# 77even/Fast-nnUNet

Hardware: AMD Instinct MI355X
Metric: 3d_fullres patches/sec (distilled r=2 student, sliding window, one 512^3 CT; volume resident in HBM at step start; step ends with: fp16 logits resident in HBM) (higher is better)
Workload: dtype f16

## Files before the change

fast-nnunet_amd/csrc/conv3d.hip:

```cpp
#include "fnn_device.h"
#include "conv_common.h"
#include <cstdlib>

template <int NB>
__global__ __launch_bounds__(256) void conv3d_mfma_kernel(const ConvParams p) {
    extern __shared__ __attribute__((aligned(16))) char smem[];
    const int tid = threadIdx.x, lane = tid & 63, wave = tid >> 6;

    int t = blockIdx.x;
    const int tw = t % p.tiles_w; t /= p.tiles_w;
    const int th = t % p.tiles_h; t /= p.tiles_h;
    const int td = t % p.tiles_d;
    const int n = t / p.tiles_d;
    const int cb0 = blockIdx.y * NB;

    const int od0 = td * FNN_TILE_D, oh0 = th * FNN_TILE_H, ow0 = tw * FNN_TILE_W;
    const int ID = (FNN_TILE_D - 1) * p.sd + p.kd;
    const int IH = (FNN_TILE_H - 1) * p.sh + p.kh;
    const int IW = (FNN_TILE_W - 1) * p.sw + p.kw;
    const int IVOX = ID * IH * IW;
    const int T = p.kd * p.kh * p.kw;
    const int cin_total = p.chunks * 16;

    char *sA = smem;
// ... 865 lines not shown
                for (int wres = 1; wres >= 0; --wres) {
                    if (!wres && !(p.ksteps == 5 || (p.ksteps == 14 && mb == 8))) continue;
                    const size_t lds = persist_lds_bytes(p, nb, mb, wres != 0);
                    const int per_cu = (int)((160 * 1024) / lds);
                    if (per_cu < 2) continue;
                    const int wpc = per_cu > 3 ? 3 : per_cu;
                    if (wres && mb == 8 && p.ksteps == 5 && (p.chunks == 1 || p.chunks == 2)) {
                        const int ivox4 = (3 * p.sd + p.kd) * ((FNN_TILE_H - 1) * p.sh + p.kh) * ((FNN_TILE_W - 1) * p.sw + p.kw);
                        if (ivox4 * 2 <= 4 * 256 && persist_lds_bytes(p, 1, 4, true) * 3 <= 160 * 1024) {
                            set_persist(c, 1, 4, 1, 5, p.chunks, 4, 0, 3);
                            return true;
                        }
                    }
                    set_persist(c, 1, mb, wres, p.ksteps == 5 ? 5 : wres ? 0 : 14, 0, 8, 0, wpc);
                    return true;
                }
            }
        }
        if (p.ksteps <= 14) {
            set_ldsk(c, nb, mbsel, 8);
            return true;
        }
    }
    if (!o.conv_v1 && s2_choose(p, c)) return true;
    if (!o.conv_v1 && p.ksteps <= 14) {
        const int nbs = (p.Cout / 16) % 2 == 0 ? 2 : 1;
        const int ID = (2 - 1) * p.sd + p.kd, IH = (FNN_TILE_H - 1) * p.sh + p.kh, IW = (FNN_TILE_W - 1) * p.sw + p.kw;
        const long long tiles = (long long)plan_n * ((p.Do + 1) / 2) * p.tiles_h * p.tiles_w;
        const int groups = (p.Cout / 16) / nbs;
        if (nbs == 2 && ID * IH * IW * 2 <= 12 * 256 && persist_lds_bytes(p, 2, 2, false, false, 12) <= 80 * 1024 &&
            tiles >= 8LL * (512 / groups) && 512 / groups >= 8 && p.chunks == 1 && persist_lds_bytes(p, 2, 2, true, true, 12) <= 80 * 1024) {
            set_persist(c, 2, 2, 1, 0, 1, 12, 1, 2);
            c.gx = 512 / groups;
            return true;
        }
        if (ID * IH * IW * 2 <= 16 * 256 && ldsk_lds_bytes(p, nbs, 2) <= 80 * 1024) {
            set_ldsk(c, nbs, 2, ID * IH * IW * 2 <= 8 * 256 ? 8 : 16);
            return true;
        }
    }
    if (nb == 4 && conv3d_lds_bytes(p, 4) > 160 * 1024) nb = 2;
    if (conv3d_lds_bytes(p, nb) > 160 * 1024) return false;
    c.kernel = CK_NB; c.t[0] = nb;
    snprintf(c.name, sizeof c.name, "conv3d_mfma_kernel<%d> (generic fallback)", nb);
    return true;
}

ConvOverrides ConvOverrides::from_env() {
    ConvOverrides o;
    o.conv_v1 = fnn_knob("FNN_CONV_V1") != nullptr;
    o.no_row = fnn_knob("FNN_NO_ROW") != nullptr;
    o.no_stem_row = fnn_knob("FNN_NO_STEM_ROW") != nullptr;
    o.no_zr6 = fnn_knob("FNN_NO_ZR6") != nullptr;
    o.no_zq12 = fnn_knob("FNN_NO_ZQ12") != nullptr;
    o.no_zsw = fnn_knob("FNN_NO_ZSW") != nullptr;
    o.no_zp = fnn_knob("FNN_NO_ZP") != nullptr;
    o.zp_no_half = fnn_knob("FNN_ZP_NO_HALF") != nullptr;
    o.zps_no_half = fnn_knob("FNN_ZPS_NO_HALF") != nullptr;
    if (const char *v = fnn_knob("FNN_ZR_MIN_WGS")) o.zr_min_wgs = atoi(v);
    if (const char *v = fnn_knob("FNN_FP8_LEVELS")) o.fp8_levels = atoi(v);
    return o;
}

bool conv_choose(const ThinParams &tp, const ConvOverrides &o, ConvChoice &c) {
    c = ConvChoice{};
    if (tp.fuse) {
        ConvChoice t;
        if (!thin_choose(tp, t)) return false;
        if (!row_choose(tp, o, c)) c = t;
        return true;
    }
    const ConvParams &p = tp.c;
    const unsigned long long out_item = 2ull * p.Do * p.Ho * p.Wo * p.Cout;
    unsigned long long in_item = 0;
    for (int i = 0; i < p.n_src; ++i) {
        const unsigned long long b = 2ull * p.Di * p.Hi * p.Wi * p.src[i].C;
        in_item = b > in_item ? b : in_item;
    }
    if (out_item >= (1ull << 31) || in_item >= (1ull << 32) || (long long)p.Di * p.Hi >= (1 << 24) || p.Wi >= (1 << 24)) return false;
    if (zp_choose(p, o, c) || zr_choose(p, o, c)) return true;
    c = ConvChoice{};
    return row_choose(tp, o, c) || conv_choose_linear(p, o, c);
}

int launch_conv(const ThinParams &tp_in, const ConvChoice &c, hipStream_t st) {
    if (c.kernel == CK_ROW_STEM && tp_in.Y * tp_in.Z >= (1ll << 30)) {
        ConvChoice t;
        return thin_choose(tp_in, t) ? launch_conv(tp_in, t, st) : -1;
    }
    fnn_note_kernel("%s", c.name);
    ThinParams tp = tp_in;
    ConvParams &p = tp.c;
    p.tile_d = FNN_TILE_D;
    p.tiles_d = (p.Do + FNN_TILE_D - 1) / FNN_TILE_D;
    p.tiles_h = (p.Ho + FNN_TILE_H - 1) / FNN_TILE_H;
    p.tiles_w = (p.Wo + FNN_TILE_W - 1) / FNN_TILE_W;
    switch (c.kernel) {
        case CK_ZS: case CK_ZSP: case CK_ZSW: case CK_ZR: case CK_ZR8: case CK_ZQ12: case CK_ZR12: case CK_ZRW:
            return launch_conv3d_zr(p, c, st);
        case CK_ZP: case CK_ZPS: return launch_conv2d_zp(p, c, st);
        case CK_ROW: case CK_ROW_STEM: return launch_conv_row(tp, c, st);
        case CK_THIN: return launch_conv_thin(tp, c, st);
        case CK_PERSIST: return launch_persist(p, c, st);
        case CK_LDSK:
            if (c.t[1] == 2) {
                if (c.t[2] == 8) return c.t[0] == 2 ? launch_ldsk<2, 2, 8>(p, st) : launch_ldsk<1, 2, 8>(p, st);
// ... 10 lines not shown
```

fast-nnunet_amd/csrc/conv3d_zr.hip:

```cpp
#include "fnn_device.h"
#include "conv_common.h"
#include <type_traits>
#include <cstdlib>

int conv3d_ksteps(int packing, int taps) { return packing == FNN_PACK_ZR ? 15 : packing == FNN_PACK_ZP ? 9 : (taps + 1) / 2; }

int conv3d_kstep_tap(int packing, int ks, int half, int taps) {
    if (packing == FNN_PACK_ZR) {
        const int pr = ks / 3, dz = ks % 3, t = 2 * pr + half;
        return t < 9 ? dz * 9 + t : -1;
    }
    const int t = 2 * ks + half;
    return t < taps ? t : -1;
}

int conv3d_pack_cout(int packing, int nblk, int cb, int m) {
    if ((packing != FNN_PACK_ZR && packing != FNN_PACK_ZP) || nblk % 2 != 0) return cb * 16 + m;
    return (cb >> 1) * 32 + (m >> 2) * 8 + (cb & 1) * 4 + (m & 3);
}

bool zr_choose(const ConvParams &p, const ConvOverrides &o, ConvChoice &c) {
    if (p.kd != 3 || p.kh != 3 || p.kw != 3 || p.sd != 1) return false;
    const int nblk = p.Cout / 16;
    const int plan_n = p.plan_N > 0 ? p.plan_N : p.N;
    c.packing = FNN_PACK_ZR; c.ksteps = 15; c.chunks = p.chunks;
    if (p.sh == 2 && p.sw == 2) {
        if (p.fp8 || nblk % 2 != 0 || (long long)p.Di * p.Hi * p.Wi >= (1 << 23) || p.Do < 8) return false;
        const int tiles_d = (p.Do + 7) / 8, tiles_h = (p.Ho + 3) / 4, tiles_w = (p.Wo + 7) / 8, groups = nblk / 2;
        if ((long long)plan_n * tiles_d * tiles_h * tiles_w * (p.Cout / 32) < 768) return false;
        c.stats_slots = tiles_d * tiles_h * tiles_w;
        const bool persistent = p.chunks == 1 && p.n_src == 1 && plan_n * c.stats_slots >= 512 * 8;
        if (persistent && !o.no_zsw && tiles_d >= 4) {
            const long long cols = (long long)plan_n * tiles_h * tiles_w * groups;
            int segs = 1;
            while (cols * segs < 8 * 512 && segs * 2 <= tiles_d / 2) segs *= 2;
            c.tps = (tiles_d + segs - 1) / segs;
            c.segs = (tiles_d + c.tps - 1) / c.tps;
            c.kernel = CK_ZSW;
            snprintf(c.name, sizeof c.name, "conv3d_zsw_kernel");
        } else if (persistent) {
            c.gx = 512 / groups < 8 ? 8 : 512 / groups;
            c.kernel = CK_ZSP;
            snprintf(c.name, sizeof c.name, "conv3d_zsp_kernel");
        } else {
            c.kernel = CK_ZS; c.t[0] = 2;
            snprintf(c.name, sizeof c.name, "conv3d_zs_kernel<2>");
        }
        return true;
    }
    if (p.sh != 1 || p.sw != 1) return false;
    const long long vox = (long long)p.Do * p.Ho * p.Wo;
    if (vox >= (1 << 23)) return false;
    if (vox * 32 * (p.chunks > 0 ? p.chunks : 1) >= (1ll << 31) || vox * 2 * p.Cout >= (1ll << 31)) return false;
    const int nb = nblk % 2 == 0 ? 2 : 1;
    const int th = (p.Ho + 7) / 8, tw = (p.Wo + 7) / 8;
    if (nb == 2 && !p.fp8 && p.Ho <= 6 && p.Wo <= 8 && p.Do >= 10 && p.Do % 10 == 0 && !o.no_zr6 &&
        (long long)plan_n * (p.Do / 10) * (nblk / 2) >= 160) {
        c.stats_slots = ((p.Do + 9) / 10) * th * tw;
        c.kernel = CK_ZR; c.t[0] = 2; c.t[1] = 10; c.t[2] = 6;
        snprintf(c.name, sizeof c.name, "conv3d_zr_kernel<%d,%d,%d>", 2, 10, 6);
        return true;
    }
    int td = 8;
    while (td >= 4 && (p.Do < td || (long long)plan_n * ((p.Do + td - 1) / td) * th * tw * (nblk / nb) < o.zr_min_wgs)) td -= 4;
    if (td < 4) return false;
    c.stats_slots = ((p.Do + td - 1) / td) * th * tw;
    c.t[0] = nb; c.t[1] = td;
    if (p.fp8) {
        c.kernel = CK_ZR8;
        snprintf(c.name, sizeof c.name, "conv3d_zr8_kernel<%d,%d>", nb, td);
    } else if (nb == 2 && !o.no_zq12 && conv3d_zq12_fits(p, c.stats_slots)) {
        c.kernel = CK_ZQ12;
        snprintf(c.name, sizeof c.name, "conv3d_zq12_kernel");
    } else if (nb == 2 && p.Ho > 8 && p.Ho <= 12 && p.Wo > 8 && p.Wo <= 12 && c.stats_slots >= (p.Do + 3) / 4) {
        c.kernel = CK_ZR12; c.t[0] = 4;
        snprintf(c.name, sizeof c.name, "conv3d_zr12_kernel<%d>", 4);
    } else if (p.chunks == 1 && td == 8 && (p.Do + 7) / 8 >= 4) {
        const int tiles_d = (p.Do + 7) / 8;
        const long long cols = (long long)plan_n * th * tw * (nblk / nb);
        int segs = 1;
        while (cols * segs < 2 * 768 && segs * 2 <= tiles_d / 2) segs *= 2;
        c.tps = (tiles_d + segs - 1) / segs;
        c.segs = (tiles_d + c.tps - 1) / c.tps;
        c.kernel = CK_ZRW;
        snprintf(c.name, sizeof c.name, "conv3d_zrw_kernel<%d>", nb);
    } else {
        c.kernel = CK_ZR;
        snprintf(c.name, sizeof c.name, "conv3d_zr_kernel<%d,%d>", nb, td);
    }
    return true;
}

typedef int fnn_i32x4 __attribute__((ext_vector_type(4)));
template <int TD, bool BIAS = true>
static __device__ __forceinline__ void zr_epilogue_pair(const ConvParams &p, const f32x4 (&acc)[TD][2], const float4 (&bv)[2],
                                                        int n, int od0, int oh0, int ow0, int cb0, int wave, int lane,
                                                        float (&t1)[2][4], float (&t2)[2][4]) {
    const int q = lane >> 4, r = lane & 15;
    const unsigned item_bytes = (unsigned)p.Do * p.Ho * p.Wo * p.Cout * 2;
    const __amdgpu_buffer_rsrc_t rsrc = __builtin_amdgcn_make_buffer_rsrc(p.out + (size_t)n * (item_bytes >> 1), 0,
                                                                           item_bytes, 0x00020000);
    const unsigned ovs2 = (unsigned)FNN_OVS(p) * 2;
    const unsigned coff = (unsigned)(cb0 + (q >> 1)) * (unsigned)(FNN_OCS(p) * 2) + (unsigned)(q & 1) * 16;
    const int oh = oh0 + 2 * wave + (r >> 3), ow = ow0 + (r & 7);
    const bool ok_hw = oh < p.Ho && ow < p.Wo;
    const f16x2 ones = {(f16)1.f, (f16)1.f};
#pragma unroll
    for (int mb = 0; mb < TD; mb += 2) {
        f16x8 o[2];
#pragma unroll
        for (int h = 0; h < 2; ++h) {
            const int od = od0 + mb + h;
            const bool ok = ok_hw && od < p.Do;
            unsigned voff = ok ? (unsigned)((od * p.Ho + oh) * p.Wo + ow) * ovs2 + coff : 0x80000000u;
#ifdef FNN_TMODE
            if (p.tmode & 4) voff = 0x80000000u;
#endif
#pragma unroll
            for (int nb = 0; nb < 2; ++nb) {
                o[h][nb * 4 + 0] = (f16)(BIAS ? acc[mb + h][nb][0] + bv[nb].x : acc[mb + h][nb][0]);
                o[h][nb * 4 + 1] = (f16)(BIAS ? acc[mb + h][nb][1] + bv[nb].y : acc[mb + h][nb][1]);
                o[h][nb * 4 + 2] = (f16)(BIAS ? acc[mb + h][nb][2] + bv[nb].z : acc[mb + h][nb][2]);
                o[h][nb * 4 + 3] = (f16)(BIAS ? acc[mb + h][nb][3] + bv[nb].w : acc[mb + h][nb][3]);
            }
            __builtin_amdgcn_raw_buffer_store_b128(__builtin_bit_cast(fnn_i32x4, o[h]), rsrc, voff, 0, 0);
            if (!ok) o[h] = (f16x8){0, 0, 0, 0, 0, 0, 0, 0};
        }
#pragma unroll
        for (int nb = 0; nb < 2; ++nb)
#pragma unroll
            for (int j = 0; j < 4; ++j) {
                const f16x2 pr = {o[0][nb * 4 + j], o[1][nb * 4 + j]};
                t1[nb][j] = __builtin_amdgcn_fdot2(pr, ones, t1[nb][j], false);
                t2[nb][j] = __builtin_amdgcn_fdot2(pr, pr, t2[nb][j], false);
            }
    }
}

typedef unsigned fnn_u32x4v __attribute__((ext_vector_type(4)));
template <int NB, int TD, int TH = 8>
__global__ __launch_bounds__(TH * 32, 2) void conv3d_zr_kernel(const ConvParams p) {
    extern __shared__ __attribute__((aligned(16))) char smem[];
    const int tid = threadIdx.x, lane = tid & 63, wave = __builtin_amdgcn_readfirstlane(tid >> 6);
    FNN_STAMP_DECL
    FNN_STAMP();
    constexpr int NT = TH * 32;
    constexpr int IH = TH + 2, IW = 10, PW = 12, ID = TD + 2;
    constexpr int PS = IH * PW * 32;
    constexpr int ABYTES = ID * PS;
    constexpr int KS = 15;
    constexpr int WB = KS * 64;
    constexpr int WPB = (WB + NT - 1) / NT;
    static_assert(WB - (WPB - 1) * NT == 192, "the last weight element group covers exactly waves 0 .. 2");

    int t;
    {
        const int nwg = gridDim.x, bid = blockIdx.x;
        const int qd = nwg >> 3, rm = nwg & 7, xcd = bid & 7, idx = bid >> 3;
        t = __builtin_amdgcn_readfirstlane((xcd < rm ? xcd * (qd + 1) : rm * (qd + 1) + (xcd - rm) * qd) + idx);
    }
    const int tw = __builtin_amdgcn_readfirstlane(t % p.tiles_w); t = __builtin_amdgcn_readfirstlane(t / p.tiles_w);
    const int th = __builtin_amdgcn_readfirstlane(t % p.tiles_h); t = __builtin_amdgcn_readfirstlane(t / p.tiles_h);
    const int td = __builtin_amdgcn_readfirstlane(t % p.tiles_d);
    const int n = __builtin_amdgcn_readfirstlane(t / p.tiles_d);
    const int cb0 = blockIdx.y * NB;
    const int od0 = td * TD, oh0 = th * 8, ow0 = tw * 8;

    char *sA = smem;
    char *sW = smem + ABYTES;

    const int col = tid >> 1, cg = tid & 1;
    const int zh = (col * 205) >> 11, zw = col - zh * IW;
    const bool has_col = tid < 2 * IH * IW;
    const int gh = oh0 - 1 + zh, gw = ow0 - 1 + zw;
    const bool ok_hw = has_col & ((unsigned)gh < (unsigned)p.Hi) & ((unsigned)gw < (unsigned)p.Wi);
    const int hw_lin = __mul24(gh, p.Wi) + gw;
    const int ldso0 = (zh * PW + zw) * 32 + ((cg ^ (zh & 1)) * 16);
    const int wlds = ABYTES + tid * 16;
    unsigned pmask = (1u << ID) - 1;
    if (od0 == 0) pmask &= ~1u;
    {
        const int over = od0 + TD + 1 - p.Di;
        if (over > 0) pmask &= (1u << (ID - over)) - 1;
    }
    pmask = __builtin_amdgcn_readfirstlane(pmask);

    f32x4 acc[TD][NB];
    fnn_u32x4v xr[ID], wr[NB][WPB];
#ifdef FNN_NORM_FP32
    float scu[16], shu[16];
#else
    fnn_u32x4v ssv[2];
#endif
    float slope_next = 1.f;
#ifdef FNN_TMODE
    bool first_chunk = true;
#endif

    __amdgpu_buffer_rsrc_t rx, rw[NB];
    unsigned voff = 0x80000000u, plane_bytes = 0;
    auto prep = [&](int ch) {
        const int c_glob = ch * 16;
        const int s = (c_glob < p.src[0].C) ? 0 : 1;
        const int c_uni = c_glob - (s ? p.src[0].C : 0);
        const int sC = p.src[s].C;
        const int vs = FNN_VS(p.src[s]);
        const unsigned item_bytes = (unsigned)p.Di * p.Hi * p.Wi * sC * 2;
        const f16 *sp = p.src[s].ptr + (size_t)n * (item_bytes >> 1) + (c_uni >> 4) * FNN_CS(p.src[s]);
        rx = __builtin_amdgcn_make_buffer_rsrc((void *)sp, 0, item_bytes, 0x00020000);
        slope_next = p.src[s].slope;
#ifdef FNN_NORM_FP32
        const float *qs = p.src[s].ss ? p.src[s].ss + (size_t)(2 * n) * sC + c_uni : p.ident_ss + c_uni;
        const float *qh = p.src[s].ss ? qs + sC : p.ident_ss + 512 + c_uni;
#pragma unroll
        for (int j = 0; j < 16; ++j) { scu[j] = qs[j]; shu[j] = qh[j]; }
#else
        {
            const unsigned short *q = p.src[s].ssh ? p.src[s].ssh + ((size_t)n * sC + c_uni) * 2 : p.ident_ssh + c_uni * 2;
            const fnn_u32x4v *qv = (const fnn_u32x4v *)(q + cg * 16);
            ssv[0] = qv[0]; ssv[1] = qv[1];
        }
#endif
        voff = ok_hw ? (unsigned)hw_lin * (unsigned)(vs * 2) + cg * 16 : 0x80000000u;
        plane_bytes = (unsigned)p.Hi * p.Wi * vs * 2;
#pragma unroll
        for (int nb = 0; nb < NB; ++nb) {
            const f16 *wp = p.wpk + ((size_t)((cb0 + nb) * p.chunks + ch) * WB) * 8;
            rw[nb] = __builtin_amdgcn_make_buffer_rsrc((void *)wp, 0, WB * 16, 0x00020000);
        }
    };
#ifndef FNN_ZR_SLICES
#define FNN_ZR_SLICES 5
#endif
    constexpr int SL = FNN_ZR_SLICES;
    auto load_part = [&](int part) {
#pragma unroll
        for (int u = 0; u < ID; ++u) {
            if (u * SL / ID != part) continue;
            int gd = od0 - 1 + u;
            gd = gd < 0 ? 0 : (gd >= p.Di ? p.Di - 1 : gd);
            xr[u] = __builtin_bit_cast(fnn_u32x4v, __builtin_amdgcn_raw_buffer_load_b128(rx, voff, (unsigned)gd * plane_bytes, 0));
        }
#ifdef FNN_TMODE
        if ((p.tmode & 8) && !first_chunk) return;
#endif
#pragma unroll
        for (int e = 0; e < NB * WPB; ++e) {
            if (e * SL / (NB * WPB) != part) continue;
            const int nb = e / WPB, u = e % WPB;
            wr[nb][u] = __builtin_bit_cast(fnn_u32x4v, __builtin_amdgcn_raw_buffer_load_b128(rw[nb], tid * 16, u * (NT * 16), 0));
        }
    };
    auto commit = [&]() {
        const f16 slope_h = (f16)slope_next;
#ifdef FNN_NORM_FP32
        float sc[8], sh[8];
#pragma unroll
        for (int j = 0; j < 8; ++j) {
            sc[j] = ok_hw ? (cg ? scu[8 + j] : scu[j]) : 0.f;
            sh[j] = ok_hw ? (cg ? shu[8 + j] : shu[j]) : 0.f;
        }
#else
        const fnn_u32x4v zero4 = {0u, 0u, 0u, 0u};
        const f16x8 sc_h = __builtin_bit_cast(f16x8, ok_hw ? ssv[0] : zero4), sh_h = __builtin_bit_cast(f16x8, ok_hw ? ssv[1] : zero4);
#endif
        if (has_col) {
#pragma unroll
            for (int u = 0; u < ID; ++u) {
                const f16x8 x = __builtin_bit_cast(f16x8, xr[u]);
#ifdef FNN_NORM_FP32
                f16x8 o;
#pragma unroll
                for (int j = 0; j < 8; ++j) o[j] = (f16)fmaf((float)x[j], sc[j], sh[j]);
#else
                f16x8 o = x * sc_h + sh_h;
#endif
                o = __builtin_elementwise_max(o, o * slope_h);
                *(f16x8 *)(sA + ldso0 + u * PS) = o;
            }
            if (pmask != (1u << ID) - 1) {
                unsigned pm = pmask;
                asm volatile("" : "+s"(pm));
#pragma unroll
                for (int u = 0; u < ID; ++u)
                    if (!((pm >> u) & 1)) *(f16x8 *)(sA + ldso0 + u * PS) = (f16x8){0, 0, 0, 0, 0, 0, 0, 0};
            }
        }
#ifdef FNN_TMODE
        if ((p.tmode & 8) && !first_chunk) return;
#endif
#pragma unroll
        for (int nb = 0; nb < NB; ++nb)
#pragma unroll
            for (int u = 0; u < WPB; ++u)
                if (u + 1 < WPB || wave < 3) *(fnn_u32x4v *)(smem + wlds + (nb * WB + u * NT) * 16) = wr[nb][u];
    };
    int toff[5];
    auto kloop = [&](bool prefetch) {
#pragma unroll
        for (int pr = 0; pr < 5; ++pr) {
            if (prefetch && pr < SL) load_part(pr);
            const char *bp = sA + toff[pr];
            f16x8 xf[ID];
#pragma unroll
            for (int pl = 0; pl < ID; ++pl) xf[pl] = *(const f16x8 *)(bp + pl * PS);
#pragma unroll
            for (int dz = 0; dz < 3; ++dz) {
                f16x8 wf[NB];
#pragma unroll
                for (int nb = 0; nb < NB; ++nb) wf[nb] = *(const f16x8 *)(sW + ((nb * KS + pr * 3 + dz) * 64 + lane) * 16);
#pragma unroll
                for (int j = 0; j < TD; ++j)
#pragma unroll
                    for (int nb = 0; nb < NB; ++nb)
                        acc[j][nb] = __builtin_amdgcn_mfma_f32_16x16x32_f16(wf[nb], xf[j + dz], acc[j][nb], 0, 0, 0);
            }
            __builtin_amdgcn_sched_barrier(0);
        }
    };

    prep(0);
#pragma unroll
    for (int part = 0; part < SL; ++part) load_part(part);
    __builtin_amdgcn_sched_barrier(0);
    FNN_STAMP();
    {
        f32x4 b0[NB];
#pragma unroll
        for (int nb = 0; nb < NB; ++nb)
            b0[nb] = *(const f32x4 *)(p.bias + cb0 * 16 + (NB == 2 ? (lane >> 4) * 8 + nb * 4 : nb * 16 + (lane >> 4) * 4));
#pragma unroll
        for (int j = 0; j < TD; ++j)
#pragma unroll
            for (int nb = 0; nb < NB; ++nb) acc[j][nb] = b0[nb];
    }
    {
        const int r = lane & 15, hl = lane >> 5, kh = (lane >> 4) & 1;
#pragma unroll
        for (int pr = 0; pr < 5; ++pr) {
            const int tp = 2 * pr + hl < 9 ? 2 * pr + hl : 8;
            const int row = 2 * wave + (r >> 3) + tp / 3, col2 = (r & 7) + tp % 3;
            toff[pr] = (row * PW + col2) * 32 + ((kh ^ (row & 1)) * 16);
        }
    }

    commit();
#ifdef FNN_TMODE
    first_chunk = false;
#endif
    __syncthreads();
    FNN_STAMP();
    for (int ch = 0; ch + 1 < p.chunks; ++ch) {
        prep(ch + 1);
        kloop(true);
        FNN_STAMP();
        __syncthreads();
        commit();
        __syncthreads();
        FNN_STAMP();
    }
    kloop(false);
    FNN_STAMP();
    __syncthreads();

    {
        float4 bv[NB];
#pragma unroll
        for (int nb = 0; nb < NB; ++nb) bv[nb] = make_float4(0.f, 0.f, 0.f, 0.f);
        float t1[NB][4], t2[NB][4];
#pragma unroll
        for (int nb = 0; nb < NB; ++nb)
#pragma unroll
            for (int j = 0; j < 4; ++j) { t1[nb][j] = 0.f; t2[nb][j] = 0.f; }
        if constexpr (NB == 2) zr_epilogue_pair<TD, false>(p, acc, bv, n, od0, oh0, ow0, cb0, wave, lane, t1, t2);
        else tile_epilogue<NB, TD, true, false>(p, acc, bv, n, od0, oh0, ow0, cb0, wave, lane, t1, t2);
        if (p.stats_out) stats_to_global<NB, true, NB == 2, TH / 2>(p, t1, t2, (float *)smem, n, cb0, wave, lane, tid, (td * p.tiles_h + th) * p.tiles_w + tw);
    }
    FNN_STAMP();
    FNN_STAMP_FLUSH(p.dbg);
}


template <int NB>
__global__ __launch_bounds__(256, NB == 1 ? 3 : 2) void conv3d_zrw_kernel(const ConvParams p, const int segs, const int tps) {
    extern __shared__ __attribute__((aligned(16))) char smem[];
    const int tid = threadIdx.x, lane = tid & 63, wave = __builtin_amdgcn_readfirstlane(tid >> 6);
    constexpr int TD = 8, IH = 10, IW = 10, PW = 12, ID = TD + 2;
    constexpr int PS = IH * PW * 32, ABYTES = ID * PS, KS = 15, WB = KS * 64, WPB = (WB + 255) / 256;

    int t;
    {
        const int nwg = gridDim.x, bid = blockIdx.x;
        const int qd = nwg >> 3, rm = nwg & 7, xcd = bid & 7, idx = bid >> 3;
        t = __builtin_amdgcn_readfirstlane((xcd < rm ? xcd * (qd + 1) : rm * (qd + 1) + (xcd - rm) * qd) + idx);
    }
    const int tw = __builtin_amdgcn_readfirstlane(t % p.tiles_w); t = __builtin_amdgcn_readfirstlane(t / p.tiles_w);
    const int th = __builtin_amdgcn_readfirstlane(t % p.tiles_h); t = __builtin_amdgcn_readfirstlane(t / p.tiles_h);
    const int seg = __builtin_amdgcn_readfirstlane(t % segs);
    const int n = __builtin_amdgcn_readfirstlane(t / segs);
    const int td0 = seg * tps, td1 = td0 + tps < p.tiles_d ? td0 + tps : p.tiles_d;
    if (td0 >= td1) return;
    const int cb0 = blockIdx.y * NB;
    const int oh0 = th * 8, ow0 = tw * 8;

    char *sA = smem;
    char *sW = smem + ABYTES;
    auto sred_at = [&](int i) { const int k = i >> 4; return (float *)(sA + (k / IH) * PS + ((k % IH) * PW + IW) * 32) + (i & 15); };

    const int col = tid >> 1, cg = tid & 1;
    const int zh = (col * 205) >> 11, zw = col - zh * IW;
    const bool has_col = tid < 2 * IH * IW;
    const int gh = oh0 - 1 + zh, gw = ow0 - 1 + zw;
    const bool ok_hw = has_col & ((unsigned)gh < (unsigned)p.Hi) & ((unsigned)gw < (unsigned)p.Wi);
    const int hw_lin = __mul24(gh, p.Wi) + gw;
// ... 1357 lines not shown
```

fast-nnunet_amd/csrc/engine.hip:

```cpp
#include "fnn_device.h"
#include "../../include/fnn.h"

#include <cmath>
#include <cstdarg>
#include <cstdlib>
#include <cstdio>
#include <cstring>
#include <string>
#include <algorithm>
#include <climits>
#include <vector>
#include <thread>

namespace {

thread_local std::string g_err;

struct Layer {
    enum Type { STEM, CONV, TCONV, POOL, COMBINE, GATHER } type;
    int n_src = 1;
    int cin_real[2] = {0, 0}, cin_pad[2] = {0, 0};
    int cout_real = 0, cout_pad = 0;
    int k[3] = {1, 1, 1}, s[3] = {1, 1, 1};
    int in_dims[3], out_dims[3];
// ... 413 lines not shown
            }
            L.packing = L.cc.packing; L.chunks = L.cc.chunks; L.ksteps = L.cc.ksteps;
            L.w_off = wpk; wpk += (size_t)(L.cout_pad / 16) * L.chunks * L.ksteps * 512;
        } else if (L.type == Layer::TCONV) {
            const int taps = L.s[0] * L.s[1] * L.s[2];
            L.ksteps = (L.cin_pad[0] + 31) / 32;
            L.w_off = wpk; wpk += (size_t)taps * (L.cout_pad / 16) * L.ksteps * 512;
        }
        L.bias_off = fp; fp += L.cout_pad;
        if (L.fp8) { L.oscale_off = fp; fp += L.cout_pad; }
        if (L.has_norm) { L.gamma_off = fp; fp += L.cout_pad; L.beta_off = fp; fp += L.cout_pad; }
        L.stats_slots = FNN_STAT_REPL;
        if (L.type == Layer::STEM) L.stats_slots = stem_mfma_stats_slots(L.out_dims[0], L.out_dims[1], L.out_dims[2]);
        else if (L.type == Layer::CONV) L.stats_slots = L.cc.stats_slots;
        L.stats_off = st; if (L.has_norm) st += (size_t)L.stats_slots * L.cout_pad * 2;
        L.ss_off = ssn; if (L.has_norm) ssn += L.cout_pad;
        L.out_off = act; act += ovox * L.cout_pad;
        flops += L.flops;
        bytes += 2.0 * ovox * L.cout_real * 2.0;
    }
    e->hblocks = (a.num_heads + 1 + 15) / 16;
    e->head_ksteps = (pad16(a.features[0]) + 31) / 32;
    e->head_w_off = wpk; wpk += (size_t)e->hblocks * e->head_ksteps * 512;
    e->head_bias_off = fp; fp += (size_t)e->hblocks * 16;
    e->n_gpass = (a.num_heads + 62) / 63;
    if (e->n_gpass > 1) {
        e->gpass_w_off = wpk; wpk += (size_t)e->n_gpass * 4 * 512;
        e->gpass_bias_off = fp; fp += (size_t)e->n_gpass * 64;
    }
    const double P = (double)a.patch[0] * a.patch[1] * a.patch[2];
    e->head_flops = 2.0 * a.num_heads * a.features[0] * P;
    e->patch_flops = flops + e->head_flops;
    for (int s = 0; s < a.n_stages - 1; ++s) {
        const Layer &L = e->layers[enc_last[s]];
        bytes += (double)L.out_dims[0] * L.out_dims[1] * L.out_dims[2] * L.cout_real * 2.0;
    }
    e->patch_act_bytes = bytes;
    e->wpk_halves = wpk; e->fparam_floats = fp; e->stats_doubles = st; e->act_halves = act; e->ss_count = ssn;
    return 0;
}

inline uint16_t f2h_bits(float f) { f16 h = (f16)f; uint16_t b; memcpy(&b, &h, 2); return b; }

void pack_conv(const Layer &L, const float *W, uint16_t *dst) {
    const int T = L.k[0] * L.k[1] * L.k[2];
    const int cin_tot = L.cin_real[0] + (L.n_src > 1 ? L.cin_real[1] : 0);
    const int nblk = L.cout_pad / 16;
    for (int cb = 0; cb < nblk; ++cb)
        for (int ch = 0; ch < L.chunks; ++ch)
            for (int ks = 0; ks < L.ksteps; ++ks)
                for (int lane = 0; lane < 64; ++lane)
                    for (int j = 0; j < 8; ++j) {
                        const int k = 8 * (lane >> 4) + j;
                        const int tap = conv3d_kstep_tap(L.packing, ks, k >> 4, T), c = ch * 16 + (k & 15);
                        const int co = conv3d_pack_cout(L.packing, nblk, cb, lane & 15);
                        int src = 0, cl = c;
                        if (c >= L.cin_pad[0]) { src = 1; cl = c - L.cin_pad[0]; }
                        float v = 0.f;
                        if (tap >= 0 && co < L.cout_real && cl < L.cin_real[src]) {
                            const int ci = (src ? L.cin_real[0] : 0) + cl;
                            v = W[((size_t)co * cin_tot + ci) * T + tap];
                        }
                        dst[((((size_t)cb * L.chunks + ch) * L.ksteps + ks) * 64 + lane) * 8 + j] = f2h_bits(v);
                    }
}

uint8_t f2e4m3(float f) {
    const uint8_t sign = std::signbit(f) ? 0x80 : 0;
    float a = std::fabs(f);
    if (!(a == a)) return sign | 0x7f;
    if (a >= 448.f) return sign | 0x7e;
    if (a < 0x1p-6f) {
        const int q = (int)std::nearbyint(a * 512.f);
        return sign | (uint8_t)q;
    }
    int e;
    const float m = std::frexp(a, &e);
    int q = (int)std::nearbyint(m * 16.f);
    int E = e - 1;
    if (q == 16) { q = 8; ++E; }
    if (E > 8 || (E == 8 && q > 14)) return sign | 0x7e;
    return sign | (uint8_t)(((E + 7) << 3) | (q - 8));
}

#define FNN_FP8_ACT_MULT 8.0f
void pack_conv_fp8(const Layer &L, const float *W, uint8_t *dst, float *scales) {
    const int T = L.k[0] * L.k[1] * L.k[2];
    const int cin_tot = L.cin_real[0] + (L.n_src > 1 ? L.cin_real[1] : 0);
    const int nblk = L.cout_pad / 16;
    std::vector<float> inv(L.cout_pad, 0.f);
    for (int co = 0; co < L.cout_pad; ++co) {
        float mx = 0.f;
        if (co < L.cout_real)
            for (size_t i = 0; i < (size_t)cin_tot * T; ++i) mx = std::max(mx, std::fabs(W[(size_t)co * cin_tot * T + i]));
        const float ws = mx > 0.f ? mx / 448.f : 1.f;
        inv[co] = 1.f / ws;
        scales[co] = ws / FNN_FP8_ACT_MULT;
    }
    for (int cb = 0; cb < nblk; ++cb)
        for (int ch = 0; ch < L.chunks; ++ch)
            for (int ks = 0; ks < L.ksteps; ++ks)
                for (int lane = 0; lane < 64; ++lane)
                    for (int j = 0; j < 8; ++j) {
                        const int k = 8 * (lane >> 4) + j;
                        const int tap = conv3d_kstep_tap(L.packing, ks, k >> 4, T), c = ch * 16 + (k & 15);
                        const int co = conv3d_pack_cout(L.packing, nblk, cb, lane & 15);
                        int src = 0, cl = c;
                        if (c >= L.cin_pad[0]) { src = 1; cl = c - L.cin_pad[0]; }
                        float v = 0.f;
                        if (tap >= 0 && co < L.cout_real && cl < L.cin_real[src]) {
                            const int ci = (src ? L.cin_real[0] : 0) + cl;
                            v = W[((size_t)co * cin_tot + ci) * T + tap] * inv[co];
                        }
                        dst[((((size_t)cb * L.chunks + ch) * L.ksteps + ks) * 64 + lane) * 8 + j] = f2e4m3(v);
                    }
}

void pack_tconv(const Layer &L, const float *W, uint16_t *dst) {
    const int taps = L.s[0] * L.s[1] * L.s[2];
    const int nblk = L.cout_pad / 16;
    for (int tap = 0; tap < taps; ++tap)
        for (int cb = 0; cb < nblk; ++cb)
            for (int ks = 0; ks < L.ksteps; ++ks)
                for (int lane = 0; lane < 64; ++lane)
                    for (int j = 0; j < 8; ++j) {
                        const int ci = ks * 32 + 8 * (lane >> 4) + j, co = cb * 16 + (lane & 15);
                        float v = 0.f;
                        if (ci < L.cin_real[0] && co < L.cout_real) v = W[((size_t)ci * L.cout_real + co) * taps + tap];
                        dst[((((size_t)tap * nblk + cb) * L.ksteps + ks) * 64 + lane) * 8 + j] = f2h_bits(v);
                    }
}

void pack_head(int heads, int cin, int hblocks, int ksteps, const float *W, uint16_t *dst) {
    for (int hb = 0; hb < hblocks; ++hb)
        for (int ks = 0; ks < ksteps; ++ks)
            for (int lane = 0; lane < 64; ++lane)
                for (int j = 0; j < 8; ++j) {
                    const int ci = ks * 32 + 8 * (lane >> 4) + j, h = hb * 16 + (lane & 15);
                    float v = 0.f;
                    if (ci < cin && h < heads) v = W[(size_t)h * cin + ci];
                    dst[(((size_t)hb * ksteps + ks) * 64 + lane) * 8 + j] = f2h_bits(v);
                }
}

enum { FAM_CONV = 0, FAM_STEM, FAM_TCONV, FAM_HEAD, FAM_FINAL };

struct Scope {
    fnn_engine *e; hipStream_t st; int idx = -1;
    Scope(fnn_engine *e_, hipStream_t st_, int family, double flops, double bytes = 0) : e(e_), st(st_) {
        fnn_klog_target(e->profiling ? &e->klog : nullptr);
        if (!e->profiling) return;
        if (e->ev_used == e->evs.size()) {
            fnn_engine::Ev ev{};
            if (hipEventCreate(&ev.a) != hipSuccess || hipEventCreate(&ev.b) != hipSuccess) return;
            e->evs.push_back(ev);
        }
        idx = (int)e->ev_used++;
        e->evs[idx].family = family; e->evs[idx].flops = flops; e->evs[idx].bytes = bytes;
// ... 1421 lines not shown
```

fast-nnunet_amd/csrc/fnn_device.h:

```cpp
#pragma once
#include <hip/hip_runtime.h>
#include <stdint.h>

typedef _Float16 f16;
typedef f16 f16x8 __attribute__((ext_vector_type(8)));
typedef f16 f16x4 __attribute__((ext_vector_type(4)));
typedef f16 f16x2 __attribute__((ext_vector_type(2)));
typedef float f32x4 __attribute__((ext_vector_type(4)));
typedef float f32x16 __attribute__((ext_vector_type(16)));

#define FNN_STAT_REPL 8
#define FNN_TILE_D 4
#define FNN_TILE_H 8
#define FNN_TILE_W 8

struct SrcDesc {
    const f16 *ptr;
    int C;
    const float *ss;
    float slope;
    int vs;
    long long cs;
    const unsigned short *ssh;
};
#define FNN_VS(S) ((S).vs ? (S).vs : (S).C)
#define FNN_CS(S) ((S).vs ? (S).cs : 16LL)
#define FNN_OVS(P) ((P).out_vs ? (P).out_vs : (P).Cout)
#define FNN_OCS(P) ((P).out_vs ? (P).out_cs : 16LL)

struct ConvParams {
    SrcDesc src[2];
    int n_src;
    int N, Di, Hi, Wi;
    int plan_N;
    int Do, Ho, Wo;
    int Cout;
    int kd, kh, kw, sd, sh, sw, pd, ph, pw;
    const f16 *wpk;
    const float *bias;
    f16 *out;
    int out_vs;
    long long out_cs;
    double *stats_out;
    int tiles_d, tiles_h, tiles_w;
    int tile_d;
    unsigned long long *dbg;
    int tmode;
    int chunks;
    int ksteps;
    const float *ident_ss;
    const unsigned short *ident_ssh;
    int packing;
    int fp8;
    const float *oscale;
    float act_mult;
    int stats_slots;
};

#define FNN_PACK_LINEAR 0
#define FNN_PACK_ZR 1
#define FNN_PACK_ZP 2
int conv_zp_chunks(int cin_pad0, int cin_pad1);
void conv_zp_pack(const float *W, int cout_real, int cout_pad, int cin_real0, int cin_pad0, int cin_real1, int cin_pad1, unsigned short *dst);

struct StemParams {
    const float *vol;
    long long vol_batch_stride;
    int C;
    long long X, Y, Z;
    const int *origins;
    int flip_d, flip_h, flip_w;
    int PD, PH, PW;
    int kd, kh, kw;
    int Cout;
    const float *w;
    const float *bias;
    f16 *out;
    double *stats_out;
    int tiles_d, tiles_h, tiles_w;
};

#define FUSE_STEM 1
#define FUSE_TCONV 2
struct ThinParams {
    ConvParams c;
    int fuse;
    const f16 *fw;
    const float *fbias;
    const float *vol;
    long long vol_batch_stride;
    long long Y, Z;
    const int *origins;
    int flip_d, flip_h, flip_w;
    const float *fss;
    float fslope;
    SrcDesc low;
    int Dl, Hl, Wl;
    int tsd, tsh, tsw;
};

struct TconvParams {
    SrcDesc src;
    int N, Di, Hi, Wi;
    int sd, sh, sw;
    int Cout;
    const f16 *wpk;
    const float *bias;
    f16 *out;
    int out_vs;
    long long out_cs;
    int ksteps;
    int nblk;
    int row_store;
    int lds_w;
// ... 134 lines not shown
    int flip_d, flip_h, flip_w;
    int PD, PH, PW, N;
    f16 *out;
    int out_vs;
    long long out_cs;
};
int launch_patch_input(const PatchInputParams &p, hipStream_t st);

struct PoolParams {
    SrcDesc src;
    int N, Di, Hi, Wi;
    int sd, sh, sw;
    f16 *out;
    int out_vs;
    long long out_cs;
};

struct CombineParams {
    SrcDesc a;
    SrcDesc b;
    long long vox;
    int N;
    float slope;
    f16 *out;
    int out_vs;
    long long out_cs;
    f16 *pool_out;
    int D, H, W, psd, psh, psw;
    int pool_vs;
    long long pool_cs;
};

struct StatsFinalizeParams {
    const double *stats;
    int nrep;
    const float *gamma, *beta;
    float *ss;
    unsigned short *ssh;
    int C;
    float inv_count, eps;
};

int launch_stats_finalize(const StatsFinalizeParams &p, int N, hipStream_t st);
int launch_region_copy(void *feat, long long n_slots, const int *regions, int n, void *message, int PD, int PH, int PW, int C, bool pack, hipStream_t st);
int launch_fss_to_ssh(const float *fss, unsigned short *ssh, long long items, int C, hipStream_t st);
int launch_avgpool(const PoolParams &p, hipStream_t st);
int launch_combine(const CombineParams &p, hipStream_t st);
bool combine_pool_ok(int D, int H, int W, int sd, int sh, int sw);
size_t conv3d_lds_bytes(const ConvParams &p, int nb);
int conv3d_pick_nb(int nblk);
const float *conv3d_identity_ss();
const unsigned short *conv3d_identity_ssh();
int conv3d_ksteps(int packing, int taps);
int conv3d_kstep_tap(int packing, int ks, int half, int taps);
int conv3d_pack_cout(int packing, int nblk, int cb, int m);

enum ConvKernel {
    CK_NONE, CK_ZS, CK_ZSP, CK_ZSW, CK_ZR, CK_ZR8, CK_ZQ12, CK_ZR12, CK_ZRW,
    CK_ZP, CK_ZPS,
    CK_ROW, CK_ROW_STEM, CK_THIN,
    CK_PERSIST, CK_LDSK, CK_S2, CK_NB
};
struct ConvChoice {
    int kernel = CK_NONE;
    int t[7] = {};
    int packing = 0, ksteps = 0, chunks = 0, stats_slots = FNN_STAT_REPL;
    int wpc = 0;
    int gx = 0;
    int segs = 0, tps = 0;
    char name[64] = "";
};
struct ConvOverrides {
    bool conv_v1 = false;
    bool no_row = false, no_stem_row = false, no_zr6 = false, no_zq12 = false, no_zsw = false, no_zp = false;
    bool zp_no_half = false, zps_no_half = false;
    int zr_min_wgs = 480;
    int fp8_levels = -1;
    static ConvOverrides from_env();
};
bool conv_choose(const ThinParams &tp, const ConvOverrides &o, ConvChoice &c);
int launch_conv(const ThinParams &tp, const ConvChoice &c, hipStream_t st);
bool zp_choose(const ConvParams &p, const ConvOverrides &o, ConvChoice &c);
int launch_conv2d_zp(ConvParams p, const ConvChoice &c, hipStream_t st);
bool zr_choose(const ConvParams &p, const ConvOverrides &o, ConvChoice &c);
int launch_conv3d_zr(ConvParams p, const ConvChoice &c, hipStream_t st);
bool conv3d_zq12_fits(const ConvParams &p, int stats_slots);
int launch_conv3d_zq12(ConvParams p, hipStream_t st);
bool row_choose(const ThinParams &tp, const ConvOverrides &o, ConvChoice &c);
int launch_conv_row(const ThinParams &tp, const ConvChoice &c, hipStream_t st);
bool thin_choose(const ThinParams &tp, ConvChoice &c);
int launch_conv_thin(const ThinParams &tp, const ConvChoice &c, hipStream_t st);
bool s2_choose(const ConvParams &p, ConvChoice &c);
int launch_conv3d_s2(ConvParams p, const ConvChoice &c, hipStream_t st);
int launch_tconv(const TconvParams &p, hipStream_t st);
bool stem_mfma_ok(int C, int kd, int kh, int kw, int cout_pad);
int stem_mfma_stats_slots(int PD, int PH, int PW);
int stem_mfma_ksteps(int C, int taps);
bool stem_mfma_kmap(int C, int taps, int ks, int k, int *c, int *tap);
int launch_stem_mfma(const StemParams &p, const f16 *wfrag, int N, hipStream_t st);
bool gather_ok(const GatherParams &p);
int launch_gather(const GatherParams &p, hipStream_t st);
int launch_quotient_check(unsigned long long *counts, hipStream_t st);
bool stem_row_ok(const StemParams &p);
int launch_stem_row(const StemParams &p, int N, hipStream_t st);
int launch_head(const HeadParams &p, hipStream_t st);
bool launch_head_first_visit_ok(const HeadParams &p);
int launch_patch_acc(const PatchAccParams &p, hipStream_t st);
int launch_finalize(const FinalizeParams &p, hipStream_t st);
int launch_labels_from_acc(const FinalizeParams &p, void *labels, int label_u16, const int *order, hipStream_t st);
int launch_scale_output(void *out, int out_fp32, long long n, int divisor, int *inf_flag, hipStream_t st);
int launch_argmax(const void *logits, int fp32, int heads, long long nvox, void *labels, int label_u16, const int *order,
                  hipStream_t st);
int launch_pad_volume(const float *src, float *dst, int C, const long long s[3], const long long d[3],
                      const long long lo[3], hipStream_t st);
```

fast-nnunet_amd/csrc/ops_api.hip:

```cpp
#include "fnn_device.h"
#include "../../include/fnn.h"

#include <cstdio>
#include <cstring>
#include <string>
#include <vector>

namespace {

inline int pad16(int c) { return (c + 15) / 16 * 16; }
inline uint16_t f2h_bits(float f) { f16 h = (f16)f; uint16_t b; memcpy(&b, &h, 2); return b; }
inline float h2f_bits(uint16_t b) { f16 h; memcpy(&h, &b, 2); return (float)h; }

struct DevBuf {
    void *p = nullptr;
    ~DevBuf() { if (p) (void)hipFree(p); }
    bool alloc(size_t n) { return hipMalloc(&p, n ? n : 16) == hipSuccess; }
    template <class T> T *as() { return (T *)p; }
};

bool op_chunk_major(int cp) { const char *v = fnn_knob("FNN_OP_CHUNK_MAJOR"); return v && v[0] != '0' && cp > 16; }

void to_ndhwc(const float *x, int n, int c, int cp, size_t vox, std::vector<uint16_t> &out, std::vector<double> *stats, bool cm = false) {
    out.assign((size_t)n * vox * cp, 0);
// ... 52 lines not shown
}

}

static thread_local std::vector<std::string> g_op_kernels;
struct OpKlog {
    OpKlog() { g_op_kernels.clear(); fnn_klog_target(&g_op_kernels); }
    ~OpKlog() { fnn_klog_target(nullptr); }
};

extern "C" {

int fnn_op_conv3d(int device, int n, const int dims[3],
                  const float *x, int cin, const float *gamma1, const float *beta1, float slope1,
                  const float *x2, int cin2, const float *gamma2, const float *beta2, float slope2,
                  const float *w, const float *bias, int cout, const int k[3], const int stride[3],
                  float *y, double *stats_out) {
    if (!x || !w || !y || !dims || !k || !stride || n < 1 || cin < 1 || cout < 1) return FNN_E_INVALID;
    if (hipSetDevice(device) != hipSuccess) return FNN_E_HIP;
    OpKlog klog;
    const size_t vox = (size_t)dims[0] * dims[1] * dims[2];
    const int nsrc = x2 ? 2 : 1;
    SrcHolder s1, s2;
    if (!make_src(s1, x, n, cin, vox, gamma1, beta1, slope1, true)) return FNN_E_HIP;
    if (x2 && !make_src(s2, x2, n, cin2, vox, gamma2, beta2, slope2, true)) return FNN_E_HIP;
    const int cp1 = pad16(cin), cp2 = x2 ? pad16(cin2) : 0, cop = pad16(cout);
    const int T = k[0] * k[1] * k[2], cin_tot = cin + (x2 ? cin2 : 0);
    ConvParams p{};
    p.n_src = nsrc; p.src[0] = s1.d;
    if (x2) p.src[1] = s2.d; else { p.src[1] = s1.d; p.src[1].C = 0; }
    p.N = n; p.Di = dims[0]; p.Hi = dims[1]; p.Wi = dims[2];
    p.kd = k[0]; p.kh = k[1]; p.kw = k[2]; p.sd = stride[0]; p.sh = stride[1]; p.sw = stride[2];
    p.pd = (k[0] - 1) / 2; p.ph = (k[1] - 1) / 2; p.pw = (k[2] - 1) / 2;
    p.Do = (p.Di + 2 * p.pd - p.kd) / p.sd + 1; p.Ho = (p.Hi + 2 * p.ph - p.kh) / p.sh + 1; p.Wo = (p.Wi + 2 * p.pw - p.kw) / p.sw + 1;
    p.Cout = cop; p.chunks = (cp1 + cp2) / 16;
    ThinParams tp{};
    tp.c = p;
    ConvChoice cc;
    if (!conv_choose(tp, ConvOverrides::from_env(), cc)) return FNN_E_UNSUPPORTED;
    p.packing = cc.packing; p.ksteps = cc.ksteps; p.chunks = cc.chunks; p.stats_slots = cc.stats_slots;
    auto launch = [&]() { tp.c = p; return launch_conv(tp, cc, 0); };
    const size_t slots = (size_t)p.stats_slots;
    p.tiles_d = (p.Do + FNN_TILE_D - 1) / FNN_TILE_D; p.tiles_h = (p.Ho + FNN_TILE_H - 1) / FNN_TILE_H;
    p.tiles_w = (p.Wo + FNN_TILE_W - 1) / FNN_TILE_W;
    p.tile_d = FNN_TILE_D;
    std::vector<uint16_t> wp((size_t)(cop / 16) * p.chunks * p.ksteps * 512, 0);
    if (p.packing == FNN_PACK_ZP) conv_zp_pack(w, cout, cop, cin, cp1, x2 ? cin2 : 0, cp2, wp.data());
    else
    for (int cb = 0; cb < cop / 16; ++cb)
        for (int ch = 0; ch < p.chunks; ++ch)
            for (int ks = 0; ks < p.ksteps; ++ks)
                for (int lane = 0; lane < 64; ++lane)
                    for (int j = 0; j < 8; ++j) {
                        const int kk = 8 * (lane >> 4) + j, tap = conv3d_kstep_tap(p.packing, ks, kk >> 4, T), c = ch * 16 + (kk & 15);
                        const int co = conv3d_pack_cout(p.packing, cop / 16, cb, lane & 15);
                        int src = 0, cl = c;
                        if (c >= cp1) { src = 1; cl = c - cp1; }
                        const int creal = src ? cin2 : cin;
                        float v = 0.f;
                        if (tap >= 0 && co < cout && cl < creal) v = w[((size_t)co * cin_tot + (src ? cin : 0) + cl) * T + tap];
                        wp[((((size_t)cb * p.chunks + ch) * p.ksteps + ks) * 64 + lane) * 8 + j] = f2h_bits(v);
                    }
    std::vector<float> bp(cop, 0.f);
    if (bias) for (int i = 0; i < cout; ++i) bp[i] = bias[i];
    const size_t ovox = (size_t)p.Do * p.Ho * p.Wo;
    DevBuf dw, db, dout, dst;
    if (!dw.alloc(wp.size() * 2 + 1024) || !db.alloc(cop * 4) || !dout.alloc((size_t)n * ovox * cop * 2) ||
        !dst.alloc((size_t)n * slots * cop * 16)) return FNN_E_HIP;
    (void)hipMemcpy(dw.p, wp.data(), wp.size() * 2, hipMemcpyHostToDevice);
    (void)hipMemcpy(db.p, bp.data(), cop * 4, hipMemcpyHostToDevice);
    (void)hipMemset(dst.p, 0, (size_t)n * slots * cop * 16);
    (void)hipMemset(dout.p, 0, (size_t)n * ovox * cop * 2);
    p.wpk = dw.as<f16>(); p.bias = db.as<float>(); p.out = dout.as<f16>(); p.stats_out = dst.as<double>();
    const bool ocm = op_chunk_major(cop);
    if (ocm) { p.out_vs = 16; p.out_cs = 16LL * (long long)ovox; }
#ifdef FNN_STAMPS
    DevBuf ddbg;
    const size_t dbg_n = (size_t)1 << 20;
    if (!ddbg.alloc(dbg_n * 8)) return FNN_E_HIP;
    (void)hipMemset(ddbg.p, 0, dbg_n * 8);
    p.dbg = ddbg.as<unsigned long long>();
    (void)launch();
    (void)hipDeviceSynchronize();
    (void)hipMemset(dst.p, 0, (size_t)n * slots * cop * 16);
#endif
    if (fnn_knob("FNN_OP_TIME")) {
        hipEvent_t e0, e1;
        (void)hipEventCreate(&e0); (void)hipEventCreate(&e1);
        for (int i = 0; i < 2; ++i) (void)launch();
        (void)hipEventRecord(e0, 0);
        for (int i = 0; i < 30; ++i) (void)launch();
        (void)hipEventRecord(e1, 0);
        (void)hipDeviceSynchronize();
        float ms = 0.f;
        (void)hipEventElapsedTime(&ms, e0, e1);
        fprintf(stderr, "[op time] conv3d %d+%d -> %d at %dx%dx%d, N = %d: %.1f us per launch\n", cin, cin2, cout, p.Di, p.Hi, p.Wi, n, ms * (1000.f / 30.f));
        (void)hipEventDestroy(e0); (void)hipEventDestroy(e1);
        (void)hipMemset(dst.p, 0, (size_t)n * slots * cop * 16);
    }
#ifdef FNN_STAMPS
    hipEvent_t ev0, ev1;
    (void)hipEventCreate(&ev0); (void)hipEventCreate(&ev1);
    (void)hipEventRecord(ev0, 0);
#endif
    const int rc = launch();
    if (rc != 0) return rc == -1 ? FNN_E_UNSUPPORTED : FNN_E_HIP;
#ifdef FNN_STAMPS
// ... 177 lines not shown
```

Measured before the change: 3593.

## Pair the odd ninth tap across adjacent input-channel chunks in ZR conv kernel

Adds a ZRP weight packing in which the ninth (leftover) tap of each depth plane, which previously wasted half of an MFMA K-step on zeros, is shared across two consecutive 16-channel chunks. The even chunk skips that K-step and keeps its input fragment in registers, and the odd chunk runs it with both chunks' channels filled. Together these remove redundant MFMA work and weight loads. It applies to generic ZR kernels with at least two chunks and an 8-high tile. In exchange it holds extra registers for the saved input fragments, and the weight-packing indexing becomes more complex.

```diff
diff --git a/fast-nnunet_amd/csrc/conv3d.hip b/fast-nnunet_amd/csrc/conv3d.hip
--- a/fast-nnunet_amd/csrc/conv3d.hip
+++ b/fast-nnunet_amd/csrc/conv3d.hip
@@ -941,6 +941,7 @@
     o.no_row = fnn_knob("FNN_NO_ROW") != nullptr;
     o.no_stem_row = fnn_knob("FNN_NO_STEM_ROW") != nullptr;
     o.no_zr6 = fnn_knob("FNN_NO_ZR6") != nullptr;
+    o.no_zrp = fnn_knob("FNN_NO_ZRP") != nullptr;
     o.no_zq12 = fnn_knob("FNN_NO_ZQ12") != nullptr;
     o.no_zsw = fnn_knob("FNN_NO_ZSW") != nullptr;
     o.no_zp = fnn_knob("FNN_NO_ZP") != nullptr;
diff --git a/fast-nnunet_amd/csrc/conv3d_zr.hip b/fast-nnunet_amd/csrc/conv3d_zr.hip
--- a/fast-nnunet_amd/csrc/conv3d_zr.hip
+++ b/fast-nnunet_amd/csrc/conv3d_zr.hip
@@ -3,19 +3,26 @@
 #include <type_traits>
 #include <cstdlib>
 
-int conv3d_ksteps(int packing, int taps) { return packing == FNN_PACK_ZR ? 15 : packing == FNN_PACK_ZP ? 9 : (taps + 1) / 2; }
-
-int conv3d_kstep_tap(int packing, int ks, int half, int taps) {
-    if (packing == FNN_PACK_ZR) {
-        const int pr = ks / 3, dz = ks % 3, t = 2 * pr + half;
-        return t < 9 ? dz * 9 + t : -1;
+int conv3d_ksteps(int packing, int taps) {
+    return packing == FNN_PACK_ZR || packing == FNN_PACK_ZRP ? 15 : packing == FNN_PACK_ZP ? 9 : (taps + 1) / 2;
+}
+
+int conv3d_kstep_tap(int packing, int ks, int half, int taps, int ch, int chunks, int *tch) {
+    *tch = ch;
+    if (packing == FNN_PACK_ZR || packing == FNN_PACK_ZRP) {
+        const int pr = ks / 3, dz = ks % 3;
+        if (pr < 4) return dz * 9 + 2 * pr + half;
+        if (packing == FNN_PACK_ZR || (ch % 2 == 0 && ch + 1 == chunks)) return half ? -1 : dz * 9 + 8;
+        if (ch % 2 == 0) return -1;
+        *tch = ch - 1 + half;
+        return dz * 9 + 8;
     }
     const int t = 2 * ks + half;
     return t < taps ? t : -1;
 }
 
 int conv3d_pack_cout(int packing, int nblk, int cb, int m) {
-    if ((packing != FNN_PACK_ZR && packing != FNN_PACK_ZP) || nblk % 2 != 0) return cb * 16 + m;
+    if ((packing != FNN_PACK_ZR && packing != FNN_PACK_ZRP && packing != FNN_PACK_ZP) || nblk % 2 != 0) return cb * 16 + m;
     return (cb >> 1) * 32 + (m >> 2) * 8 + (cb & 1) * 4 + (m & 3);
 }
 
@@ -24,6 +31,7 @@
     const int nblk = p.Cout / 16;
     const int plan_n = p.plan_N > 0 ? p.plan_N : p.N;
     c.packing = FNN_PACK_ZR; c.ksteps = 15; c.chunks = p.chunks;
+    bool zr6_shape = false;
     if (p.sh == 2 && p.sw == 2) {
         if (p.fp8 || nblk % 2 != 0 || (long long)p.Di * p.Hi * p.Wi >= (1 << 23) || p.Do < 8) return false;
         const int tiles_d = (p.Do + 7) / 8, tiles_h = (p.Ho + 3) / 4, tiles_w = (p.Wo + 7) / 8, groups = nblk / 2;
@@ -54,8 +62,9 @@
     if (vox * 32 * (p.chunks > 0 ? p.chunks : 1) >= (1ll << 31) || vox * 2 * p.Cout >= (1ll << 31)) return false;
     const int nb = nblk % 2 == 0 ? 2 : 1;
     const int th = (p.Ho + 7) / 8, tw = (p.Wo + 7) / 8;
-    if (nb == 2 && !p.fp8 && p.Ho <= 6 && p.Wo <= 8 && p.Do >= 10 && p.Do % 10 == 0 && !o.no_zr6 &&
-        (long long)plan_n * (p.Do / 10) * (nblk / 2) >= 160) {
+    zr6_shape = nb == 2 && !p.fp8 && p.Ho <= 6 && p.Wo <= 8 && p.Do >= 10 && p.Do % 10 == 0 &&
+                (long long)plan_n * (p.Do / 10) * (nblk / 2) >= 160;
+    if (zr6_shape && !o.no_zr6) {
         c.stats_slots = ((p.Do + 9) / 10) * th * tw;
         c.kernel = CK_ZR; c.t[0] = 2; c.t[1] = 10; c.t[2] = 6;
         snprintf(c.name, sizeof c.name, "conv3d_zr_kernel<%d,%d,%d>", 2, 10, 6);
@@ -86,6 +95,7 @@
         snprintf(c.name, sizeof c.name, "conv3d_zrw_kernel<%d>", nb);
     } else {
         c.kernel = CK_ZR;
+        if (p.chunks >= 2 && !zr6_shape && !o.no_zrp) c.packing = FNN_PACK_ZRP;
         snprintf(c.name, sizeof c.name, "conv3d_zr_kernel<%d,%d>", nb, td);
     }
     return true;
@@ -187,6 +197,9 @@
 
     f32x4 acc[TD][NB];
     fnn_u32x4v xr[ID], wr[NB][WPB];
+    constexpr bool PAIR = TH == 8;
+    const bool paired = PAIR && p.packing == FNN_PACK_ZRP;
+    f16x8 xl[PAIR ? ID : 1];
 #ifdef FNN_NORM_FP32
     float scu[16], shu[16];
 #else
@@ -223,10 +236,11 @@
 #endif
         voff = ok_hw ? (unsigned)hw_lin * (unsigned)(vs * 2) + cg * 16 : 0x80000000u;
         plane_bytes = (unsigned)p.Hi * p.Wi * vs * 2;
+        const int wbytes = paired && ch % 2 == 0 && ch + 1 < p.chunks ? 12 * 64 * 16 : WB * 16;
 #pragma unroll
         for (int nb = 0; nb < NB; ++nb) {
             const f16 *wp = p.wpk + ((size_t)((cb0 + nb) * p.chunks + ch) * WB) * 8;
-            rw[nb] = __builtin_amdgcn_make_buffer_rsrc((void *)wp, 0, WB * 16, 0x00020000);
+            rw[nb] = __builtin_amdgcn_make_buffer_rsrc((void *)wp, 0, wbytes, 0x00020000);
         }
     };
 #ifndef FNN_ZR_SLICES
@@ -296,14 +310,26 @@
                 if (u + 1 < WPB || wave < 3) *(fnn_u32x4v *)(smem + wlds + (nb * WB + u * NT) * 16) = wr[nb][u];
     };
     int toff[5];
-    auto kloop = [&](bool prefetch) {
-#pragma unroll
-        for (int pr = 0; pr < 5; ++pr) {
-            if (prefetch && pr < SL) load_part(pr);
+    const bool khalf1 = lane >= 32;
+    auto kloop = [&](bool prefetch, auto mode_c) __attribute__((always_inline)) {
+        constexpr int MODE = decltype(mode_c)::value;
+#pragma unroll
+        for (int i = 0; i < 5; ++i) {
+            const int pr = MODE == 2 ? (i + 4) % 5 : i;
+            if (prefetch && i < SL) load_part(i);
             const char *bp = sA + toff[pr];
+            if (MODE == 1 && pr == 4) {
+#pragma unroll
+                for (int pl = 0; pl < ID; ++pl) xl[pl] = *(const f16x8 *)(bp + pl * PS);
+                break;
+            }
             f16x8 xf[ID];
 #pragma unroll
             for (int pl = 0; pl < ID; ++pl) xf[pl] = *(const f16x8 *)(bp + pl * PS);
+            if (MODE == 2 && pr == 4) {
+#pragma unroll
+                for (int pl = 0; pl < ID; ++pl) xf[pl] = khalf1 ? xf[pl] : xl[pl];
+            }
 #pragma unroll
             for (int dz = 0; dz < 3; ++dz) {
                 f16x8 wf[NB];
@@ -318,7 +344,6 @@
             __builtin_amdgcn_sched_barrier(0);
         }
     };
-
     prep(0);
 #pragma unroll
     for (int part = 0; part < SL; ++part) load_part(part);
@@ -350,16 +375,34 @@
 #endif
     __syncthreads();
     FNN_STAMP();
-    for (int ch = 0; ch + 1 < p.chunks; ++ch) {
+    using M0 = std::integral_constant<int, 0>;
+    using M1 = std::integral_constant<int, 1>;
+    using M2 = std::integral_constant<int, 2>;
+    auto next_chunk = [&](int ch, auto mode_c) __attribute__((always_inline)) {
         prep(ch + 1);
-        kloop(true);
+        kloop(true, mode_c);
         FNN_STAMP();
         __syncthreads();
         commit();
         __syncthreads();
         FNN_STAMP();
-    }
-    kloop(false);
+    };
+    if (PAIR && paired) {
+        int ch = 0;
+        for (; ch + 2 < p.chunks; ch += 2) {
+            next_chunk(ch, M1{});
+            next_chunk(ch + 1, M2{});
+        }
+        if (ch + 1 < p.chunks) {
+            next_chunk(ch, M1{});
+            kloop(false, M2{});
+        } else {
+            kloop(false, M0{});
+        }
+    } else {
+        for (int ch = 0; ch + 1 < p.chunks; ++ch) next_chunk(ch, M0{});
+        kloop(false, M0{});
+    }
     FNN_STAMP();
     __syncthreads();
 
diff --git a/fast-nnunet_amd/csrc/engine.hip b/fast-nnunet_amd/csrc/engine.hip
--- a/fast-nnunet_amd/csrc/engine.hip
+++ b/fast-nnunet_amd/csrc/engine.hip
@@ -489,7 +489,8 @@
                 for (int lane = 0; lane < 64; ++lane)
                     for (int j = 0; j < 8; ++j) {
                         const int k = 8 * (lane >> 4) + j;
-                        const int tap = conv3d_kstep_tap(L.packing, ks, k >> 4, T), c = ch * 16 + (k & 15);
+                        int tch;
+                        const int tap = conv3d_kstep_tap(L.packing, ks, k >> 4, T, ch, L.chunks, &tch), c = tch * 16 + (k & 15);
                         const int co = conv3d_pack_cout(L.packing, nblk, cb, lane & 15);
                         int src = 0, cl = c;
                         if (c >= L.cin_pad[0]) { src = 1; cl = c - L.cin_pad[0]; }
@@ -540,7 +541,8 @@
                 for (int lane = 0; lane < 64; ++lane)
                     for (int j = 0; j < 8; ++j) {
                         const int k = 8 * (lane >> 4) + j;
-                        const int tap = conv3d_kstep_tap(L.packing, ks, k >> 4, T), c = ch * 16 + (k & 15);
+                        int tch;
+                        const int tap = conv3d_kstep_tap(L.packing, ks, k >> 4, T, ch, L.chunks, &tch), c = tch * 16 + (k & 15);
                         const int co = conv3d_pack_cout(L.packing, nblk, cb, lane & 15);
                         int src = 0, cl = c;
                         if (c >= L.cin_pad[0]) { src = 1; cl = c - L.cin_pad[0]; }
diff --git a/fast-nnunet_amd/csrc/fnn_device.h b/fast-nnunet_amd/csrc/fnn_device.h
--- a/fast-nnunet_amd/csrc/fnn_device.h
+++ b/fast-nnunet_amd/csrc/fnn_device.h
@@ -60,6 +60,7 @@
 #define FNN_PACK_LINEAR 0
 #define FNN_PACK_ZR 1
 #define FNN_PACK_ZP 2
+#define FNN_PACK_ZRP 3
 int conv_zp_chunks(int cin_pad0, int cin_pad1);
 void conv_zp_pack(const float *W, int cout_real, int cout_pad, int cin_real0, int cin_pad0, int cin_real1, int cin_pad1, unsigned short *dst);
 
@@ -300,7 +301,7 @@
 const float *conv3d_identity_ss();
 const unsigned short *conv3d_identity_ssh();
 int conv3d_ksteps(int packing, int taps);
-int conv3d_kstep_tap(int packing, int ks, int half, int taps);
+int conv3d_kstep_tap(int packing, int ks, int half, int taps, int ch, int chunks, int *tch);
 int conv3d_pack_cout(int packing, int nblk, int cb, int m);
 
 enum ConvKernel {
@@ -320,7 +321,7 @@
 };
 struct ConvOverrides {
     bool conv_v1 = false;
-    bool no_row = false, no_stem_row = false, no_zr6 = false, no_zq12 = false, no_zsw = false, no_zp = false;
+    bool no_row = false, no_stem_row = false, no_zr6 = false, no_zrp = false, no_zq12 = false, no_zsw = false, no_zp = false;
     bool zp_no_half = false, zps_no_half = false;
     int zr_min_wgs = 480;
     int fp8_levels = -1;
diff --git a/fast-nnunet_amd/csrc/ops_api.hip b/fast-nnunet_amd/csrc/ops_api.hip
--- a/fast-nnunet_amd/csrc/ops_api.hip
+++ b/fast-nnunet_amd/csrc/ops_api.hip
@@ -128,7 +128,9 @@
             for (int ks = 0; ks < p.ksteps; ++ks)
                 for (int lane = 0; lane < 64; ++lane)
                     for (int j = 0; j < 8; ++j) {
-                        const int kk = 8 * (lane >> 4) + j, tap = conv3d_kstep_tap(p.packing, ks, kk >> 4, T), c = ch * 16 + (kk & 15);
+                        int tch;
+                        const int kk = 8 * (lane >> 4) + j, tap = conv3d_kstep_tap(p.packing, ks, kk >> 4, T, ch, p.chunks, &tch);
+                        const int c = tch * 16 + (kk & 15);
                         const int co = conv3d_pack_cout(p.packing, cop / 16, cb, lane & 15);
                         int src = 0, cl = c;
                         if (c >= cp1) { src = 1; cl = c - cp1; }
```

Result: faster. 3661 (median of 6 runs) (+1.9%).
